# wizardyesterday/RtlSdrDiags

Measured on AMD Instinct MI355X. Metric: IQ MSamples/s through WBFM chain at 1/2/4/8 GPUs; % HBM roofline, higher is better.
Workload: dtype int8/int16 Q15 + f32; 1 GPU; BASELINE configs[1]: WBFM, 1 channel, 2^28-sample synthetic IQ; channels_per_gpu=1, log2_samples_per_channel=28, kernels=streaming pipelines

## Files before the change

### include/iqdemod.h

```cpp
#ifndef IQDEMOD_H
#define IQDEMOD_H

#include <stddef.h>
#include <stdint.h>

#ifdef __cplusplus
extern "C" {
#endif

#define IQD_ABI_VERSION 1

enum iqd_mode {
    IQD_MODE_NONE = 0, IQD_MODE_AM = 1, IQD_MODE_FM = 2,
    IQD_MODE_WBFM = 3, IQD_MODE_LSB = 4, IQD_MODE_USB = 5
};

enum iqd_demod { IQD_DEMOD_AM = 1, IQD_DEMOD_FM = 2, IQD_DEMOD_WBFM = 3, IQD_DEMOD_SSB = 4 };

enum iqd_status {
    IQD_OK = 0,
    IQD_EINVAL = -1,
    IQD_ENODEV = -2,
    IQD_ENOMEM = -3,
    IQD_EHIP = -4,
// ... 80 lines not shown

int iqd_demod_accept(iqd_t *e, uint32_t first_ch, uint32_t n_ch, int demod,
                     const int8_t *iq, size_t bytes_per_ch, int16_t *pcm);
int iqd_demod_set_sideband(iqd_t *e, uint32_t first_ch, uint32_t n_ch, int lsb);

int iqd_front_end(iqd_t *e, uint32_t first_ch, uint32_t n_ch, const uint8_t *iq, size_t bytes_per_ch, int8_t *out);
int iqd_front_end_device(iqd_t *e, uint32_t first_ch, uint32_t n_ch, const void *iq_dev, size_t bytes_per_ch,
                         void *out_dev);
int iqd_convert_fs_over_4(iqd_t *e, int direction, int8_t *buffer, size_t byte_count);

typedef struct iqd_stats {
    uint64_t accepts;
    uint64_t samples;
    uint64_t kernel_launches;
    uint64_t state_checks;
    uint64_t state_repairs;
    double chain_kernel_ms;
    uint64_t chain_kernel_count;
    uint64_t segment_repairs;
    uint64_t stream_launches;
    uint64_t device_launches;
    uint64_t device_copies;
    uint64_t mixed_launches;
} iqd_stats;

int iqd_get_stats(iqd_t *e, iqd_stats *out);
int iqd_set_profiling(iqd_t *e, int enabled);
int iqd_get_channel_mode(iqd_t *e, uint32_t ch, int *mode);
int iqd_get_channel_gain(iqd_t *e, uint32_t ch, int demod, float *gain);
const char *iqd_last_error(iqd_t *e);
const char *iqd_strerror(int status);
uint32_t iqd_abi_version(void);

enum iqd_resample_kind { IQD_RESAMPLE_DECIMATE_F32 = 0, IQD_RESAMPLE_INTERPOLATE_F32 = 1, IQD_RESAMPLE_INTERPOLATE_I16 = 2 };
typedef struct iqd_resampler iqd_resampler_t;
int iqd_resampler_create(iqd_t *e, int kind, const float *taps, uint32_t n_taps, uint32_t factor, uint32_t n_channels,
                         iqd_resampler_t **out);
void iqd_resampler_destroy(iqd_resampler_t *r);
int iqd_resampler_reset(iqd_resampler_t *r);
size_t iqd_resampler_out_count(const iqd_resampler_t *r, size_t n_in);
int iqd_resampler_run(iqd_resampler_t *r, const void *in, size_t n_in, void *out);
int iqd_resampler_run_device(iqd_resampler_t *r, const void *in_dev, size_t n_in, void *out_dev);

typedef struct iqd_channelizer_config {
    uint32_t n_sources;
    uint32_t n_channels;
// ... 53 lines not shown
```

### rtlsdrdiags_amd/capi.py

```python
import ctypes as C
import os
import weakref

import numpy as np

from .build import LIB as _DEFAULT_LIB

LIB = os.environ.get("IQD_LIB", _DEFAULT_LIB)

MODE = {"none": 0, "am": 1, "fm": 2, "wbfm": 3, "lsb": 4, "usb": 5}
DEMOD = {"am": 1, "fm": 2, "wbfm": 3, "ssb": 4}
F_NO_MAGNITUDE = 0x1
F_WBFM_TILES, F_WBFM_STREAM, F_PREPASS_OVERLAP = 0x2, 0x4, 0x8


class Config(C.Structure):
    _fields_ = [("abi_version", C.c_uint32), ("n_channels", C.c_uint32), ("block_bytes", C.c_uint32),
                ("device", C.c_int32), ("flags", C.c_uint32), ("reserved", C.c_uint32 * 3)]


class Stats(C.Structure):
    _fields_ = [("accepts", C.c_uint64), ("samples", C.c_uint64), ("kernel_launches", C.c_uint64),
                ("state_checks", C.c_uint64), ("state_repairs", C.c_uint64),
                ("chain_kernel_ms", C.c_double), ("chain_kernel_count", C.c_uint64), ("segment_repairs", C.c_uint64),
                ("stream_launches", C.c_uint64), ("device_launches", C.c_uint64), ("device_copies", C.c_uint64),
                ("mixed_launches", C.c_uint64)]


class AgcState(C.Structure):
    _fields_ = [("enabled", C.c_uint32), ("type", C.c_uint32), ("operating_point_dbfs", C.c_int32),
                ("deadband_db", C.c_uint32), ("blanking_limit", C.c_uint32), ("alpha", C.c_float),
                ("rx_gain_db", C.c_uint32), ("if_gain_db", C.c_uint32), ("filtered_if_gain_db", C.c_float),
                ("blanking_counter", C.c_uint32), ("gain_was_adjusted", C.c_uint32),
                ("normalized_level_dbfs", C.c_int32), ("signal_magnitude", C.c_uint32)]


class ChannelizerConfig(C.Structure):
    _fields_ = [("n_sources", C.c_uint32), ("n_channels", C.c_uint32), ("decimation", C.c_uint32),
                ("n_taps", C.c_uint32), ("taps", C.c_void_p), ("decimation_den", C.c_uint32),
                ("reserved", C.c_uint32 * 3)]


class IqdError(RuntimeError):
    def __init__(self, status, detail):
        super().__init__("libiqdemod: %s (%d): %s" % (_lib().iqd_strerror(status).decode(), status, detail))
        self.status = status


EXPORTS = [
# ... 552 lines not shown
```

### rtlsdrdiags_amd/csrc/iqd_accept.cpp

```cpp
#include "iqd_engine_impl.h"

extern "C" {


static void rebuild_lists(iqd_t *e, uint32_t first_ch, uint32_t n_ch)
{
    for (auto &l : e->h_lists) l.clear();
    e->any_gated = e->any_agc = false;
    for (uint32_t c = 0; c < n_ch; c++) {
        const ChanParams &p = e->h_params[first_ch + c];
        e->h_lists[family_of_mode(p.mode)].push_back(c);
        ChanParams worst = p;
        if (e->agc_touched[first_ch + c] && worst.rx_gain_db < AGC_MAX_GAIN) worst.rx_gain_db = AGC_MAX_GAIN;
        if (!squelch_always_open(worst, e->consts)) e->any_gated = true;
        if (e->h_agc[first_ch + c].enabled) e->any_agc = true;
    }
    for (int f = 0; f < FAM_COUNT; f++) {
        auto &l = e->h_lists[f];
        auto grp = [&](uint32_t c) { return 1 - e->h_params[first_ch + c].rotation; };
        std::stable_sort(l.begin(), l.end(), [&](uint32_t x, uint32_t y) { return grp(x) < grp(y); });
        for (int r = 0; r < 3; r++) e->rot_count[f][r] = 0;
        for (uint32_t c : l) e->rot_count[f][grp(c)]++;
    }
    e->list_first = first_ch;
// ... 4 lines not shown
namespace {
struct CallCtx {
    uint32_t first_ch = 0, n_ch = 0;
    const void *iq_dev = nullptr;
    size_t bytes_per_ch = 0;
    void *pcm_dev = nullptr, *pcm_count_dev = nullptr, *magnitude_dev = nullptr, *signal_present_dev = nullptr;
    uint32_t call_bb = 0, call_bs = 0, n_blocks = 0, vlen = 0;
    bool gated = false, any_agc = false, want_mag = false, pre_overlap = false, fused_mag = false;
    int pre_set = -1;
    DevBuf *gate_blk = nullptr, *gate_vlen = nullptr;
    SquelchLaunch q{};
    ChainLaunch base{};
    const CallPlan *plan = nullptr;
    hipStream_t s_main = nullptr;
    bool lane_used[4] = {false, false, false, false};
    bool timed = false, evp_open = false;
    std::pair<Event, Event> evp;
    MixedStreamArgs mix{};
    bool epoch_report_now = false;
    ChainLaunch tail_a{};
    int tail_f = 0;
    bool tail_pending = false;
    bool tail_dc = false;
};

int take_event_pair(iqd_t *e, CallCtx &x, hipStream_t s)
{
    if (e->ev_free_pairs.empty()) {
        Event a0, a1;
        HIP_TRY(e, hipEventCreate(a0.put()));
        HIP_TRY(e, hipEventCreate(a1.put()));
        e->ev_free_pairs.emplace_back(std::move(a0), std::move(a1));
    }
    x.evp = std::move(e->ev_free_pairs.back());
    e->ev_free_pairs.pop_back();
    HIP_TRY(e, hipEventRecord(x.evp.first, s));
    return IQD_OK;
}
}

static int prepare_call(iqd_t *e, CallCtx &x)
{
    hipStream_t s = e->stream;
    std::lock_guard<std::mutex> lk(e->mu);
    if (e->epoch_report_pending && ((volatile uint32_t *)e->h_epoch_report)[1] == e->epoch_report_seq) {
        if (((volatile uint32_t *)e->h_epoch_report)[0] == 0u)
// ... 172 lines not shown
    HIP_TRY(e, b8.ensure((size_t)x.n_ch * x.base.pcm_stride * sizeof(int32_t)));
    a.base8k = b8.as<int32_t>();
    a.dc_tiles = (uint32_t)((x.base.pcm_stride + DC_TILE - 1) / DC_TILE);
    DevBuf &dcr = f == FAM_SSB ? e->dc_records2 : e->dc_records;
    const size_t rec_bytes = (size_t)a.n_list * a.dc_tiles * sizeof(DcRecord);
    const bool grown = dcr.cap < rec_bytes + a.n_list * sizeof(uint32_t);
    HIP_TRY(e, dcr.ensure(rec_bytes + a.n_list * sizeof(uint32_t)));
    a.dc_records = dcr.p;
    size_t (&layout)[2] = e->dcr_layout[f == FAM_SSB];
    if (grown || layout[0] != rec_bytes || layout[1] < a.n_list) {
        HIP_COPY(e, hipMemsetAsync(dcr.as<char>() + rec_bytes, 0, a.n_list * sizeof(uint32_t), s));
        layout[0] = rec_bytes;
        layout[1] = a.n_list;
    }
    return IQD_OK;
}

static int queue_family(iqd_t *e, CallCtx &x, int f)
{
    const CallPlan &plan = *x.plan;
    const FamilyPlan &fp = plan.fam[f];
    const bool fused = plan.fused, forked = plan.forked, streams = fp.path == PLAN_STREAM;
    const uint32_t n_list = (uint32_t)e->h_lists[f].size();
    hipStream_t s = fp.lane == 0 ? x.s_main : e->fam_stream[fp.lane - 1];
    if (fp.lane != 0 && !x.lane_used[fp.lane]) HIP_TRY(e, hipStreamWaitEvent(s, e->fam_fork, 0));
    x.lane_used[fp.lane] = true;

    ChainLaunch a = x.base;
    a.ch_list = e->lists[f].as<uint32_t>();
    a.n_list = n_list;
    a.tile_len = fp.tile_len;
    a.tiles_per_ch = fp.tiles_per_ch;
    if (f == FAM_WBFM && x.gated && e->wbfm_epochs_live && !e->epoch_report_pending) {
        bool any = false;
        for (uint32_t c : e->h_lists[FAM_WBFM]) any = any || e->wbfm_epoch_left[x.first_ch + c] != 0;
        if (any) {
            if (!e->h_epoch_report) HIP_TRY(e, e->h_epoch_report.alloc(2));
            ((volatile uint32_t *)e->h_epoch_report)[0] = 0u;
            a.epoch_report = e->h_epoch_report;
            e->epoch_report_channels.clear();
            for (uint32_t c : e->h_lists[FAM_WBFM]) e->epoch_report_channels.push_back(x.first_ch + c);
            x.epoch_report_now = true;
        }
    }
    if (e->profiling && !x.timed && !fused) {
        int rc = take_event_pair(e, x, s);
// ... 16 lines not shown
            StreamArgs sa = e->stream_args;
            sa.amat = e->d_amat[stream_rot + 1];
            sa.half_lut = e->d_half_lut;
            sa.n_segments = n_list * a.tiles_per_ch;
            sa.grouped = fp.grouped ? 1u : 0u;
            for (int r = 0; r < 3; r++) {
                sa.group_start[r] = fp.grouped ? fp.group_start[r] : 0u;
                sa.group_li0[r] = fp.grouped ? fp.group_li0[r] : 0u;
                sa.group_nseg[r] = fp.grouped ? fp.group_nseg[r] : 0u;
                sa.amat3[r] = e->d_amat[2 - r];
            }
            sa.group_start[3] = fp.grouped ? fp.group_start[3] : 0u;
            sa.rounds = fp.rounds;
            sa.rings = fp.rings;
            HIP_TRY(e, e->stream_hist.ensure((size_t)sa.n_segments * sizeof(StHist)));
            sa.hist = e->stream_hist.as<StHist>();
            a.verify_at_end = x.gated ? 2u : 1u;
            if (fused) {
                x.mix.a[f] = a;
                x.mix.sa = sa;
                x.mix.wbfm_rot = stream_rot;
            } else {
                HIP_LAUNCH(e, launch_wbfm_stream(a, sa, stream_rot, x.fused_mag, fp.epochs, fp.grid, s));
                HIP_LAUNCH(e, launch_wbfm_stream_fixup(a, sa, s));
            }
            if (!x.gated) e->stream_handoffs += (uint64_t)n_list * ((x.vlen + a.tile_len - 1) / a.tile_len - 1);
            e->stats.stream_launches++;
        } else {
            HIP_LAUNCH(e, launch_wbfm(a, x.gated, x.fused_mag, n_list * a.tiles_per_ch, s));
        }
    } else {
        D4Args d4 = e->d4_args;
        if (streams) {
            for (int r = 0; r < 3; r++) {
                d4.group_start[r] = fp.group_start[r];
                d4.group_li0[r] = fp.group_li0[r];
                d4.group_nseg[r] = fp.group_nseg[r];
            }
            d4.group_start[3] = fp.group_start[3];
            d4.amat = e->d_amat4 + (size_t)(f == FAM_FM ? 0 : 3) * 4 * 64 * 4;
            d4.fm_lut = e->d_fmlut;
            d4.halo = (int32_t)fp.halo;
            d4.lead_shift = fp.lead_shift;
            d4.rounds = fp.rounds;
            d4.rings = fp.rings;
        }
        if (f != FAM_FM) {
// ... 16 lines not shown
                            (x.want_mag || x.pcm_count_dev || x.signal_present_dev || e->trace_on);
                if (f != FAM_FM && !x.tail_dc) HIP_LAUNCH(e, launch_am_dc(a, f, s, true));
            }
            e->stats.stream_launches++;
        } else if (f == FAM_FM) {
            HIP_LAUNCH(e, launch_fm(a, x.gated, x.fused_mag, n_list * a.tiles_per_ch, s));
        } else {
            HIP_LAUNCH(e, launch_am(a, f, x.gated, x.fused_mag, n_list * a.tiles_per_ch, s));
        }
    }
    if (e->profiling && !x.timed && !fused) {
        x.evp_open = true;
        x.timed = true;
    }
    e->stats.kernel_launches++;
    if (fused) return IQD_OK;
    if (f == FAM_WBFM && !x.gated && e->wbfm_epochs_live)
        for (uint32_t c : e->h_lists[FAM_WBFM]) {
            uint32_t &left = e->wbfm_epoch_left[x.first_ch + c];
            if (!left) continue;
            left = left > x.vlen ? left - x.vlen : 0u;
            if (!left) e->wbfm_epochs_live--;
        }
    const bool rides_with_squelch = !forked && !x.gated && !e->demod_bypass &&
                                    (x.want_mag || x.pcm_count_dev || x.signal_present_dev || e->trace_on);
    if (f == FAM_WBFM) {
        if (!streams) HIP_LAUNCH(e, launch_wbfm_verify(a, s));
        if (rides_with_squelch) {
            x.tail_a = a;
            x.tail_f = f;
            x.tail_pending = true;
        } else {
            HIP_LAUNCH(e, launch_wbfm_repair(a, x.gated, s));
        }
    } else if (rides_with_squelch) {
        x.tail_a = a;
        x.tail_f = f;
        x.tail_pending = true;
    } else {
        HIP_LAUNCH(e, launch_tail_update(a, f, s));
    }
    return IQD_OK;
}

static int queue_commit(iqd_t *e, CallCtx &x)
{
    const CallPlan &plan = *x.plan;
    hipStream_t s = x.s_main;
// ... 6 lines not shown
        e->stats.mixed_launches++;
        MixedTailArgs mt{};
        for (int f = 0; f < FAM_COUNT; f++) mt.a[f] = x.mix.a[f];
        mt.sa = x.mix.sa;
        HIP_LAUNCH(e, launch_mixed_tail(mt, s));
        if (e->profiling) x.evp_open = true;
        if (x.mix.a[FAM_WBFM].wg_count) {
            x.tail_a = x.mix.a[FAM_WBFM];
            x.tail_f = FAM_WBFM;
            x.tail_pending = true;
        }
    }
    for (int k = 1; k < 4; k++)
        if (x.lane_used[k]) {
            HIP_TRY(e, hipEventRecord(e->fam_join[k - 1], e->fam_stream[k - 1]));
            HIP_TRY(e, hipStreamWaitEvent(s, e->fam_join[k - 1], 0));
        }

    if (x.fused_mag && !e->h_lists[FAM_COUNT].empty())
        HIP_LAUNCH(e, launch_magnitude((const uint8_t *)x.iq_dev, x.bytes_per_ch, e->lists[FAM_COUNT].as<uint32_t>(),
                                    (uint32_t)e->h_lists[FAM_COUNT].size(), x.call_bs, x.n_blocks, e->mag_sums.as<uint32_t>(), s));
    if (!x.gated && !e->demod_bypass && (x.want_mag || x.pcm_count_dev || x.signal_present_dev || e->trace_on)) {
        x.q.zero_sums_after = x.any_agc ? 0u : 1u;
        HIP_LAUNCH(e, launch_squelch(x.q, true, s, x.tail_pending ? &x.tail_a : nullptr, x.tail_f, x.tail_pending && x.tail_dc));
        x.tail_pending = false;
        if (x.q.zero_sums_after) e->mag_sums_zero = (size_t)x.n_ch * x.n_blocks;
    }
    if (x.tail_pending) {
        if (x.tail_f == FAM_WBFM) HIP_LAUNCH(e, launch_wbfm_repair(x.tail_a, x.gated, s));
        else HIP_LAUNCH(e, launch_tail_update(x.tail_a, x.tail_f, s));
    }

    if (x.evp_open) {
        HIP_TRY(e, hipEventRecord(x.evp.second, s));
        e->ev_pending.push_back(std::move(x.evp));
    }
    if (x.pre_set >= 0) {
        HIP_TRY(e, hipEventRecord(e->ev_chain_done[x.pre_set], s));
        e->chain_pending[x.pre_set] = true;
    } else if (e->pre_stream && !e->demod_bypass) {
        HIP_TRY(e, hipEventRecord(e->ev_main_decisions, s));
        e->decisions_on_main = true;
    }
    if (x.epoch_report_now) {
        HIP_LAUNCH(e, launch_write_word(e->h_epoch_report + 1, e->accept_seq, s));
        e->epoch_report_pending = true;
        e->epoch_report_seq = e->accept_seq;
// ... 311 lines not shown
```

### rtlsdrdiags_amd/csrc/iqd_engine_impl.h

```cpp
#pragma once
#include "iqdemod.h"

#include <hip/hip_runtime.h>
#include <math.h>
#include <stdarg.h>
#include <stdio.h>
#include <string.h>

#include <algorithm>
#include <mutex>
#include <string>
#include <utility>
#include <vector>

#include "iqd_hipres.h"
#include "iqd_host.h"
#include "iqd_plan.h"
#include "iqd_kernels.h"
#include "iqd_stream.h"
#include "iqd_stream_mixed.h"
#include "iqd_taps.h"
#include "iqd_wbfm.h"
#include "iqd_chains.h"

// ... 48 lines not shown
    uint32_t wbfm_epochs_live = 0;
    std::vector<int32_t> rot_applied;
    bool rot_changed = false;
    DevArray<ScanConfig> d_scan_cfg;
    DevArray<ScanState> d_scan;
    DevArray<float> d_atan, d_fmlut;
    DevArray<float> d_half_lut;
    DevArray<uint32_t> d_amat[3];
    DevArray<uint32_t> d_amat4;
    D4Args d4_args{};
    std::vector<float> fm_kmax;
    bool stream_ok = false;
    std::vector<uint32_t> mode_gen, rot_gen;
    std::vector<float> wbfm_kmax;
    StreamArgs stream_args{};
    uint64_t stream_handoffs = 0;
    DevArray<uint32_t> d_counters;
    DevArray<unsigned long long> d_stamps;
    PinnedArray<uint32_t> h_counters;

    DevBuf stream_hist;
    DevBuf lists[FAM_COUNT + 1], mag_sums, blk_lists, vlen, records, base8k, base8k2, gain_trace, freq_trace, dc_records, dc_records2, repair_flags;
    size_t mag_sums_zero = 0;
    Stream pre_stream;
    Event ev_pre_done[2], ev_chain_done[2], ev_main_decisions;
    DevBuf g_sums[2], g_blk[2], g_vlen[2];
    int gate_set = 0;
    bool chain_pending[2] = {false, false};
    bool decisions_on_main = false;
    bool in_host_path = false;
    DevBuf st_iq, st_pcm, st_count, st_mag, st_allowed;
    DevBuf sl_iq[2], sl_pcm[2], sl_count[2], sl_mag[2], sl_allowed[2];
    Stream copy_stream;
    Stream fam_stream[3];
    Event fam_fork, fam_join[3];
    Event ev_in[2], ev_free[2];
    PinnedArray<uint32_t> h_slice_counts;
    DevArray<uint32_t> d_closed;
    PinnedArray<uint32_t> h_closed;
    PinnedArray<uint8_t> h_small;

    bool profiling = false;
    std::vector<std::pair<Event, Event>> ev_free_pairs, ev_pending;
    iqd_stats stats{};
    std::string last_error;

// ... 55 lines not shown
```

### rtlsdrdiags_amd/csrc/iqd_kernels.h

```cpp
#pragma once
#include <hip/hip_runtime.h>
#include <stddef.h>
#include <stdint.h>

#include "iqd_device.h"

namespace iqd {

struct WbfmStart;
struct WbfmRecord;

enum Counter { CNT_TILE_MISMATCH = 0, CNT_TILE_CHECKS = 1, CNT_SEG_REPAIRS = 2, CNT_DC_REDO = 3, CNT_TILE_REPAIRS = 4, CNT_STREAM_MISMATCH = 5, CNT_COUNT = 8 };
constexpr uint32_t MAX_MISMATCH_LIST = 1024;

struct ChainLaunch {
    const uint8_t *iq;
    size_t ch_stride_bytes;
    const uint32_t *ch_list;
    uint32_t n_list;
    uint32_t first_ch;
    uint32_t vlen;
    const uint32_t *vlen_gated;
    const uint32_t *blk_lists;
    uint32_t n_blocks;
// ... 60 lines not shown
struct StreamArgs;
hipError_t init_wbfm_stream_kernels();
hipError_t init_d4_stream_kernels();
hipError_t launch_wbfm_stream(const ChainLaunch &a, const StreamArgs &sa, int rotation, bool mag, bool epochs, uint32_t grid, hipStream_t s);
struct D4Args;
hipError_t launch_d4_stream(const ChainLaunch &a, const D4Args &da, int mode, bool mag, uint32_t grid, hipStream_t s);
hipError_t launch_am_dc(const ChainLaunch &a, int family, hipStream_t s, bool channel_major = false);
hipError_t launch_wbfm_stream_fixup(const ChainLaunch &a, const StreamArgs &sa, hipStream_t s);
hipError_t launch_retail(uint8_t *tails, const ChanParams *params, uint32_t n_ch, hipStream_t s);
hipError_t launch_resample(int kind, const void *in, void *out, const void *hist, void *hist_next, const void *taps,
                           uint32_t n_ch, uint32_t n_in, uint32_t n_out, uint32_t hist_len, uint32_t n_taps,
                           uint32_t factor, uint32_t first, hipStream_t s);
hipError_t launch_wbfm_repair(const ChainLaunch &a, bool gated, hipStream_t s);
hipError_t launch_front_end(const uint8_t *iq, int8_t *out, const ChanParams *params, uint32_t first_ch, uint32_t n_ch,
                            size_t bytes_per_ch, hipStream_t s);
hipError_t launch_rotate_signed(int8_t *buf_dev, size_t bytes, int rotation, hipStream_t s);
hipError_t launch_agc_apply(const AgcConfig *cfg, AgcState *st, const ScanConfig *scfg, ScanState *sst,
                            ChanParams *params, GainEpoch *epochs, uint32_t n_ch, hipStream_t s);
hipError_t launch_tail_update(const ChainLaunch &a, int family, hipStream_t s);
hipError_t launch_write_word(uint32_t *word, uint32_t value, hipStream_t s);
hipError_t launch_magnitude(const uint8_t *iq, size_t ch_stride_bytes, const uint32_t *ch_list, uint32_t n_list,
                            uint32_t block_samples, uint32_t n_blocks, uint32_t *mag_sums, hipStream_t s);
hipError_t launch_squelch(const SquelchLaunch &q, bool always_open, hipStream_t s, const ChainLaunch *tail_of = nullptr, int tail_family = 0, bool tail_dc = false);
hipError_t launch_tile_fill(uint8_t *dst, size_t period, size_t total, hipStream_t s);

}
```

### rtlsdrdiags_amd/csrc/iqd_kernels.hip

```cpp
#include <hip/hip_runtime.h>

#include "iqd_kernels.h"
#include "iqd_chains.h"
#include "iqd_wbfm.h"
#include "iqd_stream_fix.h"

namespace iqd {

__constant__ Consts g_consts;

hipError_t upload_consts(const Consts &c, hipStream_t s)
{
    return hipMemcpyToSymbolAsync(HIP_SYMBOL(g_consts), &c, sizeof(Consts), 0, hipMemcpyHostToDevice, s);
}

hipError_t consts_address(const Consts **p)
{
    void *a = nullptr;
    const hipError_t e = hipGetSymbolAddress(&a, HIP_SYMBOL(g_consts));
    *p = (const Consts *)a;
    return e;
}

struct DeviceExec {
// ... 101 lines not shown
#endif
template <bool GATED, bool MAG>
__global__ __launch_bounds__(WB_THREADS, IQD_WBFM_MIN_WAVES) void wbfm_chain_kernel(const ChainLaunch a)
{
    __shared__ WbfmLds lds;
    const uint32_t li = blockIdx.x / a.tiles_per_ch, tile = blockIdx.x - li * a.tiles_per_ch;
    const uint32_t ch = a.ch_list[li];
    const uint32_t vlen = GATED ? a.vlen_gated[ch] : a.vlen;
    if ((int64_t)tile * a.tile_len >= (int64_t)vlen) return;
    WbfmStart start;
    if (tile == 0) {
        const WbfmCarry cy = a.wbfm_carry[a.first_ch + ch];
        start.y = cy.y; start.u = cy.u; start.back = cy.back; start.cold = 0;
    } else {
        start.y = 0.f; start.u = 0.f; start.back = 0; start.cold = 1;
    }
    wbfm_run_tile<GATED, MAG>(a, lds, li, tile, ch, vlen, start);
}

__device__ __forceinline__ void tail_update_body(const ChainLaunch &a, int family, uint32_t li);
static_assert(WB_THREADS == 256, "the repair kernel ends with the tail update, which moves 16 bytes per thread");

template <bool GATED>
__device__ __forceinline__ void wbfm_repair_body(const ChainLaunch &a, WbfmLds &lds, const uint32_t li)
{
    const uint32_t ch = a.ch_list[li];
    const uint32_t vlen = GATED ? a.vlen_gated[ch] : a.vlen;
    const uint32_t ntiles = (vlen + a.tile_len - 1) / a.tile_len;
    if (a.verify_at_end == 2 && threadIdx.x == 0 && ntiles > 1) atomicAdd(&a.counters[CNT_TILE_CHECKS], ntiles - 1);
    if (!a.repair_flags[li]) {
        tail_update_body(a, FAM_WBFM, li);
        return;
    }
    WbfmRecord *r = a.records + (size_t)li * a.tiles_per_ch;
    const bool strong = a.params[a.first_ch + ch].wbfm_k >= 1.0f;
    __shared__ uint32_t first_bad;
    uint32_t from = 1;
    for (;;) {
        if (threadIdx.x == 0) first_bad = ntiles;
        __syncthreads();
        for (uint32_t tile = from + threadIdx.x; tile < ntiles; tile += blockDim.x)
            if (!iir_states_agree(r[tile].y_in, a.verify_at_end ? r[tile - 1].y_end : r[tile - 1].y_out, strong)) {
                atomicMin(&first_bad, tile);
                break;
            }
        __syncthreads();
        uint32_t tile = first_bad;
        __syncthreads();
        if (tile >= ntiles) break;
        bool redo_next = false;
        for (; tile < ntiles; tile++) {
            const WbfmRecord prev = r[tile - 1];
            const bool ok = iir_states_agree(r[tile].y_in, a.verify_at_end ? prev.y_end : prev.y_out, strong);
            if (ok && !redo_next) break;
            redo_next = a.verify_at_end && !ok;
            if (a.verify_at_end && tile + 2 == ntiles && vlen - (ntiles - 1) * a.tile_len < (uint32_t)FORCED_BACK) redo_next = true;
            WbfmStart start;
            start.y = prev.y_out; start.u = prev.u_out; start.back = prev.back_out; start.cold = 0;
            wbfm_run_tile<GATED, false>(a, lds, li, tile, ch, vlen, start);
            __threadfence();
            __syncthreads();
            if (threadIdx.x == 0) atomicAdd(&a.counters[CNT_TILE_REPAIRS], 1u);
        }
        from = tile;
        if (from >= ntiles) break;
    }
    if (threadIdx.x == 0) a.repair_flags[li] = 0;
    tail_update_body(a, FAM_WBFM, li);
}

template <bool GATED>
__global__ __launch_bounds__(WB_THREADS, IQD_WBFM_MIN_WAVES) void wbfm_repair_kernel(const ChainLaunch a)
{
    __shared__ WbfmLds lds;
    wbfm_repair_body<GATED>(a, lds, blockIdx.x);
}

__device__ __forceinline__ bool setup_tile(const ChainLaunch &a, bool gated, int family, Tile &t, uint32_t &ch, uint32_t &ech)
{
    const uint32_t li = blockIdx.x / a.tiles_per_ch, tile = blockIdx.x - li * a.tiles_per_ch;
    ch = a.ch_list[li];
    ech = a.first_ch + ch;
    const uint32_t vlen = gated ? a.vlen_gated[ch] : a.vlen;
    const int64_t v0 = (int64_t)tile * a.tile_len;
    if (v0 >= (int64_t)vlen) return false;
    const ChanParams &p = a.params[ech];
    t.iq_ch = a.iq + (size_t)ch * a.ch_stride_bytes;
    t.tail = a.tails + ((size_t)ech * FAM_COUNT + family) * TAIL_BYTES;
    t.blk_list = gated ? a.blk_lists + (size_t)ch * a.n_blocks : nullptr;
    t.block_samples = a.block_samples;
// ... 165 lines not shown
    }
}

__global__ void wbfm_verify_kernel(const ChainLaunch a)
{
    const uint32_t idx = blockIdx.x * blockDim.x + threadIdx.x;
    const uint32_t li = idx / a.tiles_per_ch, tile = idx % a.tiles_per_ch;
    if (li >= a.n_list) return;
    const uint32_t ch = a.ch_list[li];
    const uint32_t vlen = a.vlen_gated ? a.vlen_gated[ch] : a.vlen;
    const uint32_t ntiles = (vlen + a.tile_len - 1) / a.tile_len;
    if (tile >= ntiles) return;
    const WbfmRecord *r = a.records + (size_t)li * a.tiles_per_ch;
    if (tile > 0) {
        if (!iir_states_agree(r[tile].y_in, a.verify_at_end ? r[tile - 1].y_end : r[tile - 1].y_out, a.params[a.first_ch + ch].wbfm_k >= 1.0f)) {
            atomicAdd(&a.counters[CNT_TILE_MISMATCH], 1u);
            a.repair_flags[li] = 1;
        } else {
            atomicAdd(&a.counters[CNT_TILE_CHECKS], 1u);
        }
    }
}

__device__ __forceinline__ void tail_update_body(const ChainLaunch &a, int family, uint32_t li)
{
    const uint32_t ch = a.ch_list[li];
    const uint32_t ech = a.first_ch + ch;
    const uint32_t vlen = a.vlen_gated ? a.vlen_gated[ch] : a.vlen;
    if (family == FAM_WBFM && a.epoch_report && threadIdx.x == 0 &&
        (uint64_t)a.epochs[ech].wbfm.since[0] + vlen < (uint64_t)TAIL)
        *(volatile uint32_t *)a.epoch_report = 1u;
    if (vlen == 0) return;
    if (family == FAM_WBFM && threadIdx.x == 0) {
        const uint32_t ntiles = (vlen + a.tile_len - 1) / a.tile_len;
        const WbfmRecord r = a.records[(size_t)li * a.tiles_per_ch + ntiles - 1];
        const WbfmRecord p = a.records[(size_t)li * a.tiles_per_ch + (ntiles >= 2 ? ntiles - 2 : 0)];
        a.wbfm_carry[ech] = wbfm_pick_carry(r, p, ntiles, vlen, a.tile_len, a.verify_at_end);
    }
    if (threadIdx.x < EPOCHS && (family == FAM_WBFM || family == FAM_FM)) {
        uint32_t *since = (family == FAM_WBFM ? a.epochs[ech].wbfm.since : a.epochs[ech].fm.since) + threadIdx.x;
        const uint64_t total = (uint64_t)*since + vlen;
        *since = total < (uint64_t)TAIL ? (uint32_t)total : (uint32_t)TAIL;
    }
    uint8_t *tail = a.tails + ((size_t)ech * FAM_COUNT + family) * TAIL_BYTES;
    const uint8_t *iq_ch = a.iq + (size_t)ch * a.ch_stride_bytes;
    const uint32_t *blk_list = a.vlen_gated ? a.blk_lists + (size_t)ch * a.n_blocks : nullptr;
    const int keep = family == FAM_WBFM ? tail_keep(FAM_WBFM) : family == FAM_FM ? tail_keep(FAM_FM) : family == FAM_AM ? tail_keep(FAM_AM) : tail_keep(FAM_SSB);
    const bool mine = 8 * (int)threadIdx.x < keep;
    const int64_t v = (int64_t)vlen - keep + 8 * (int64_t)(mine ? threadIdx.x : 0);
    const uint8_t *src;
    if (v < 0) src = tail + TAIL_BYTES + 2 * v;
    else if (!blk_list) src = iq_ch + 2 * v;
    else {
        const uint32_t blk = (uint32_t)(v / a.block_samples);
        const uint32_t off = (uint32_t)(v - (int64_t)blk * a.block_samples);
        src = iq_ch + ((int64_t)blk_list[blk] * a.block_samples + off) * 2;
    }
    uint4 val{};
    if (mine) val = *(const uint4 *)src;
    __syncthreads();
#ifndef IQD_NO_WT_STORES
// ... 60 lines not shown
{
    if (blockIdx.x < a.n_list) tail_update_body(a, family, blockIdx.x);
    else squelch_block_body(q, always_open, (blockIdx.x - a.n_list) * 256u + threadIdx.x);
}

__global__ __launch_bounds__(256) void tail_dc_squelch_kernel(const ChainLaunch a, int family, const SquelchLaunch q, int always_open)
{
    __shared__ DcLds lds;
    if (blockIdx.x < a.n_list) {
        if (threadIdx.x >= 64) return;
        dc_channel_wave(a, family, blockIdx.x, lds);
    } else if (blockIdx.x < 2 * a.n_list) {
        tail_update_body(a, family, blockIdx.x - a.n_list);
    } else {
        squelch_block_body(q, always_open, (blockIdx.x - 2 * a.n_list) * 256u + threadIdx.x);
    }
}

__global__ __launch_bounds__(WB_THREADS, IQD_WBFM_MIN_WAVES) void wbfm_repair_squelch_kernel(const ChainLaunch a, const SquelchLaunch q, int always_open)
{
    __shared__ WbfmLds lds;
    if (blockIdx.x < a.n_list) wbfm_repair_body<false>(a, lds, blockIdx.x);
    else squelch_block_body(q, always_open, (blockIdx.x - a.n_list) * 256u + threadIdx.x);
}

struct MixedTailRoles { uint32_t end[6]; };
__global__ __launch_bounds__(256) void mixed_tail_kernel(const ChainLaunch a_wbfm, const StreamArgs sa, const ChainLaunch a_am,
                                                         const ChainLaunch a_fm, const ChainLaunch a_ssb, const MixedTailRoles roles)
{
    __shared__ union Lds { DcLds dc; FixLds fix; __device__ Lds() {} } u;
    DcLds &lds = u.dc;
    const uint32_t b = blockIdx.x;
    if (b < roles.end[0]) {
        wbfm_stream_fixup_body(a_wbfm, sa, b, u.fix);
    } else if (b < roles.end[2]) {
        if (threadIdx.x >= 64) return;
        const int family = b < roles.end[1] ? FAM_AM : FAM_SSB;
        const ChainLaunch &a = family == FAM_AM ? a_am : a_ssb;
        const uint32_t li = b - (family == FAM_AM ? roles.end[0] : roles.end[1]);
        dc_channel_wave(a, family, li, lds);
    } else if (b < roles.end[3]) {
        tail_update_body(a_am, FAM_AM, b - roles.end[2]);
    } else if (b < roles.end[4]) {
        tail_update_body(a_fm, FAM_FM, b - roles.end[3]);
    } else if (b < roles.end[5]) {
        tail_update_body(a_ssb, FAM_SSB, b - roles.end[4]);
// ... 445 lines not shown
}

hipError_t launch_tail_update(const ChainLaunch &a, int family, hipStream_t s)
{
    hipLaunchKernelGGL(tail_update_kernel, dim3(a.n_list), dim3(256), 0, s, a, family);
    return hipGetLastError();
}

__global__ void write_word_kernel(uint32_t *word, uint32_t value) { *(volatile uint32_t *)word = value; }
hipError_t launch_write_word(uint32_t *word, uint32_t value, hipStream_t s)
{
    hipLaunchKernelGGL(write_word_kernel, dim3(1), dim3(1), 0, s, word, value);
    return hipGetLastError();
}

hipError_t launch_magnitude(const uint8_t *iq, size_t ch_stride_bytes, const uint32_t *ch_list, uint32_t n_list,
                            uint32_t block_samples, uint32_t n_blocks, uint32_t *mag_sums, hipStream_t s)
{
    hipLaunchKernelGGL(magnitude_kernel, dim3(n_blocks, n_list), dim3(256), 0, s, iq, ch_stride_bytes, ch_list,
                       block_samples, n_blocks, mag_sums);
    return hipGetLastError();
}

hipError_t launch_squelch(const SquelchLaunch &q, bool always_open, hipStream_t s, const ChainLaunch *tail_of, int tail_family, bool tail_dc)
{
    const uint32_t n = q.n_ch * q.n_blocks;
    if (tail_of && tail_dc)
        hipLaunchKernelGGL(tail_dc_squelch_kernel, dim3(2 * tail_of->n_list + (n + 255) / 256), dim3(256), 0, s, *tail_of, tail_family, q, always_open ? 1 : 0);
    else if (tail_of && tail_family == FAM_WBFM)
        hipLaunchKernelGGL(wbfm_repair_squelch_kernel, dim3(tail_of->n_list + (n + 255) / 256), dim3(WB_THREADS), 0, s, *tail_of, q, always_open ? 1 : 0);
    else if (tail_of)
        hipLaunchKernelGGL(tail_squelch_kernel, dim3(tail_of->n_list + (n + 255) / 256), dim3(256), 0, s, *tail_of, tail_family, q, always_open ? 1 : 0);
    else
        hipLaunchKernelGGL(squelch_block_kernel, dim3((n + 255) / 256), dim3(256), 0, s, q, always_open ? 1 : 0);
    if (!always_open || q.any_agc) {
        if (q.n_blocks >= 32)
            hipLaunchKernelGGL(squelch_track_wave_kernel, dim3(q.n_ch), dim3(64), 0, s, q, always_open ? 1 : 0);
        else
            hipLaunchKernelGGL(squelch_track_kernel, dim3((q.n_ch + 63) / 64), dim3(64), 0, s, q, always_open ? 1 : 0);
    }
    return hipGetLastError();
}

hipError_t launch_mixed_tail(const MixedTailArgs &m, hipStream_t s)
{
    MixedTailRoles roles;
    uint32_t at = 0;
    if (m.a[FAM_WBFM].wg_count) at += (m.sa.n_segments + FIX_SEGS - 1) / FIX_SEGS;
    roles.end[0] = at;
    if (m.a[FAM_AM].wg_count) at += m.a[FAM_AM].n_list;
    roles.end[1] = at;
    if (m.a[FAM_SSB].wg_count) at += m.a[FAM_SSB].n_list;
    roles.end[2] = at;
    if (m.a[FAM_AM].wg_count) at += m.a[FAM_AM].n_list;
    roles.end[3] = at;
    if (m.a[FAM_FM].wg_count) at += m.a[FAM_FM].n_list;
    roles.end[4] = at;
    if (m.a[FAM_SSB].wg_count) at += m.a[FAM_SSB].n_list;
    roles.end[5] = at;
    if (at) hipLaunchKernelGGL(mixed_tail_kernel, dim3(at), dim3(256), 0, s, m.a[FAM_WBFM], m.sa, m.a[FAM_AM], m.a[FAM_FM], m.a[FAM_SSB], roles);
    return hipGetLastError();
}

// ... 47 lines not shown
```

### rtlsdrdiags_amd/csrc/iqd_plan.cpp

```cpp
#include "iqd_plan.h"

#include <algorithm>

#include "iqdemod.h"
#include "iqd_stream.h"

namespace iqd {

uint64_t stream_min_seg(const PlanKnobs &k, int f, uint64_t vlen, int several_families)
{
    if (k.env_stream_min_seg) return k.env_stream_min_seg;
    if (several_families == 2) return STREAM_MIN_SEG_FORKED;
    if (several_families) return vlen < 8192 ? STREAM_MIN_SEG_MIXED_SHORT : STREAM_MIN_SEG_MIXED;
    if (f == FAM_WBFM) return STREAM_MIN_SEG_WBFM;
    if (f == FAM_FM) return STREAM_MIN_SEG_FM;
    if (f == FAM_AM) return vlen <= 16384 ? STREAM_MIN_SEG_AM_SHORT : STREAM_MIN_SEG_AM;
    return vlen <= 16384 ? STREAM_MIN_SEG_SSB_SHORT : STREAM_MIN_SEG_SSB;
}

namespace {

uint32_t halo_of(int f, uint32_t shift)
{
    return f == FAM_WBFM ? (uint32_t)ST_HALO : (uint32_t)d4_full_halo(f) - shift;
}

uint32_t group_ids(const FamilyShape &s, FamilyPlan &p)
{
    uint32_t at = 0, li0 = 0;
    for (int r = 0; r < 3; r++) {
        p.group_start[r] = at;
        p.group_li0[r] = li0;
        p.group_nseg[r] = s.rot_count[r] * p.tiles_per_ch;
        at += (p.group_nseg[r] + 15u) / 16u * 16u;
        li0 += s.rot_count[r];
    }
    p.group_start[3] = at;
    return at;
}

// ... 153 lines not shown
                    }
                    if (!shift || k.d4_leadfree >= 0 || p.tiles_per_ch >= D4_LEADFREE_MIN_TILES) break;
                    shift = 0;
                }
            }
        }
        if (fused) {
            if (p.path != PLAN_STREAM) return false;
            p.wg_first = out.mix_wgs;
            out.mix_wgs += p.grid;
        }
    }
    return true;
}

}

void plan_call(const PlanKnobs &k, const CallShape &c, CallPlan &out)
{
    if (!plan_once(k, c, true, out)) plan_once(k, c, false, out);
}

}
```

### rtlsdrdiags_amd/csrc/iqd_stream.h

```cpp
#pragma once
#include <stdint.h>

#include "iqd_device.h"

namespace iqd {

constexpr int ST_WAVES = 15;
constexpr int ST_THREADS = 64 * ST_WAVES;
constexpr int ST_RINGS = 3;
constexpr int ST_P_PER_RING = 4;
constexpr int ST_SEGS = 64 * ST_RINGS;
constexpr int ST_HALO = FORCED_BACK;
#ifndef IQD_ST_AHEAD
#define IQD_ST_AHEAD 2
#endif
constexpr int ST_AHEAD = IQD_ST_AHEAD;
constexpr int ST_MIN_TILE = 768;
constexpr int ST_FIX_PCM = 21;
constexpr int ST_ROW_FLOATS = 260;
#ifndef IQD_ST_FAKE_SHIFT
#define IQD_ST_FAKE_SHIFT 0
#endif
constexpr int ST_LDS_ROW_FLOATS = IQD_ST_FAKE_SHIFT ? (256 >> IQD_ST_FAKE_SHIFT) + 4 : ST_ROW_FLOATS;
constexpr int ST_TABLE_BYTES = 129 * ST_LDS_ROW_FLOATS * 4;
// ... 18 lines not shown
    uint32_t y2_last[20];
};
static_assert(sizeof(StHist) == 256, "one boundary record per segment, 256 bytes");

struct StreamArgs {
    StHist *hist;
    const uint32_t *amat;
    const float *half_lut;
    uint32_t n_segments;
    uint32_t rounds;
    uint32_t rings;
    uint32_t grouped;
    uint32_t group_start[4];
    uint32_t group_li0[3];
    uint32_t group_nseg[3];
    const uint32_t *amat3[3];
    uint32_t d1p[4];
    uint32_t d1p2[4];
    uint32_t p12p[6];
    uint32_t a40p[20];
    float b0, a1;
};

enum { D4_AM = 0, D4_SSB = 1, D4_FM = 2 };
constexpr int D4_HALO_AM = fir_halo(FAM_AM), D4_HALO_SSB = fir_halo(FAM_SSB), D4_HALO_FM = fir_halo(FAM_FM);
constexpr int D4_HALO_SHORT = 128;
constexpr int d4_full_halo(int family) { return family == FAM_FM ? D4_HALO_FM : family == FAM_AM ? D4_HALO_AM : D4_HALO_SSB; }
constexpr int d4_lead_shift(int family) { return d4_full_halo(family) - D4_HALO_SHORT; }
constexpr int D4_REPLAY_AM = 4, D4_REPLAY_SSB = 36, D4_REPLAY_FM = 20;
constexpr int D4_REPLAY_PAIRS_AMSSB = 4;
constexpr int D4_RAILS_FROM_PIECE = 8;
constexpr int d4_replay_outputs(int family) { return family == FAM_FM ? D4_REPLAY_FM : family == FAM_AM ? D4_REPLAY_AM : D4_REPLAY_SSB; }
struct D4Geom { int64_t v0; uint32_t skip, cold; };
#if defined(__HIPCC__)
__host__ __device__
#endif
inline D4Geom d4_geom(uint32_t sid, uint32_t tile, uint32_t tile_len, uint32_t shift)
{
    D4Geom g;
    if (!shift) { g.v0 = (int64_t)tile * tile_len; g.skip = 0; g.cold = 1; return g; }
    g.cold = tile == 0 || (sid & 63u) == 0 ? 1u : 0u;
    const uint32_t c = 1u + (sid >> 6) - ((sid - tile) >> 6);
    g.v0 = (int64_t)tile * tile_len - (int64_t)shift * c;
    g.skip = g.cold ? shift : 0u;
    return g;
}
// ... 24 lines not shown
```

### rtlsdrdiags_amd/csrc/iqd_stream_fix.h

```cpp
#pragma once
#include <hip/hip_runtime.h>

#include "iqd_kernels.h"
#include "iqd_stream.h"
#include "iqd_stream_mixed.h"
#include "iqd_wbfm.h"
#include "iqd_mfma.h"

namespace iqd {

struct StSeg {
    uint32_t valid, li, tile, ch, ech;
    int32_t v0, tlen;
    int32_t vlen;
};

__device__ __forceinline__ StSeg st_segment(const ChainLaunch &a, uint32_t sid, uint32_t n_segments)
{
    StSeg s;
    s.valid = sid < n_segments ? 1u : 0u;
    const uint32_t id = s.valid ? sid : 0u;
    s.li = id / a.tiles_per_ch;
    s.tile = id - s.li * a.tiles_per_ch;
    s.ch = a.ch_list[s.li];
// ... 73 lines not shown
#pragma unroll
        for (int k = 0; k < 4; k++) y1[k] = prev.y1_last[k];
#pragma unroll
        for (int k = 0; k < 6; k++) y1[4 + k] = own.y1_first[k];
        y1[4] = (y1[4] & 0xffff0000u) | ((uint32_t)(acc >> 15) & 0xffffu);
        int s2 = 1 << 14;
#pragma unroll
        for (int q = 0; q < 6; q++) {
            const uint32_t d = i == 0 ? y1[5 - q] : (i == 1 ? y1[7 - q] : y1[9 - q]);
            s2 = dot2(d, sa.p12p[q], s2);
        }
        ((int16_t *)&y2x[sl][20])[i] = (int16_t)(s2 >> 15);
    } else if (live) {
        for (int p = i - 3; p < 41; p += FIX_LANES - 3) {
            if (p == 20) continue;
            if (p == 21) ((int16_t *)&y2x[sl][21])[1] = (int16_t)(own.y2_first[1] >> 16);
            else y2x[sl][p] = p < 20 ? prev.y2_last[p] : own.y2_first[p - 20];
        }
    }
    if (live && i == FIX_LANES - 1 && f2u(y_in) != f2u(y_end)) {
        if (!iir_states_agree(y_in, y_end, a.params[sg.ech].wbfm_k >= 1.0f)) {
            atomicAdd(&a.counters[CNT_TILE_MISMATCH], 1u);
            atomicAdd(&a.counters[CNT_STREAM_MISMATCH], 1u);
            a.repair_flags[sg.li] = 1;
        }
    }
    __syncthreads();
    if (!live) return;
    for (int j = i; j < ST_FIX_PCM && j < sg.tlen / 32; j += FIX_LANES) {
        int s3 = 1 << 14;
#pragma unroll
        for (int q = 0; q < 20; q++) {
            const uint32_t pair = y2x[sl][20 + j - q];
            s3 = clamp_q30(dot2(pair, sa.a40p[q] & 0xffff0000u, s3));
            s3 = clamp_q30(dot2(pair, sa.a40p[q] & 0x0000ffffu, s3));
        }
        a.pcm[(size_t)sg.ch * a.pcm_stride + (sg.v0 >> 5) + j] = (int16_t)(s3 >> 15);
    }
}

}
```

Before: 829,300 MSamples/s.

## Fuse WBFM stream fixup, tail update and squelch into one closing kernel

For up to eight WBFM channels where a squelch pass follows, the separate stream fixup launch and the squelch/tail launch are merged into one kernel. Workgroups take fixup, tail-update or squelch roles, and a striped atomic arrival counter picks the last workgroup. That workgroup re-runs the repair walk against saved old tails when any channel was flagged. This removes a kernel launch and its inter-kernel gap per call, at the cost of extra atomics, a tail snapshot store, and a serial repair path in a single workgroup when repair is needed.

```diff
diff --git a/include/iqdemod.h b/include/iqdemod.h
--- a/include/iqdemod.h
+++ b/include/iqdemod.h
@@ -126,6 +126,7 @@
     uint64_t device_launches;
     uint64_t device_copies;
     uint64_t mixed_launches;
+    uint64_t closed_in_fixup;
 } iqd_stats;
 
 int iqd_get_stats(iqd_t *e, iqd_stats *out);
diff --git a/rtlsdrdiags_amd/capi.py b/rtlsdrdiags_amd/capi.py
--- a/rtlsdrdiags_amd/capi.py
+++ b/rtlsdrdiags_amd/capi.py
@@ -24,7 +24,7 @@
                 ("state_checks", C.c_uint64), ("state_repairs", C.c_uint64),
                 ("chain_kernel_ms", C.c_double), ("chain_kernel_count", C.c_uint64), ("segment_repairs", C.c_uint64),
                 ("stream_launches", C.c_uint64), ("device_launches", C.c_uint64), ("device_copies", C.c_uint64),
-                ("mixed_launches", C.c_uint64)]
+                ("mixed_launches", C.c_uint64), ("closed_in_fixup", C.c_uint64)]
 
 
 class AgcState(C.Structure):
diff --git a/rtlsdrdiags_amd/csrc/iqd_accept.cpp b/rtlsdrdiags_amd/csrc/iqd_accept.cpp
--- a/rtlsdrdiags_amd/csrc/iqd_accept.cpp
+++ b/rtlsdrdiags_amd/csrc/iqd_accept.cpp
@@ -50,6 +50,8 @@
     int tail_f = 0;
     bool tail_pending = false;
     bool tail_dc = false;
+    bool close_in_fixup = false;
+    StreamArgs close_sa{};
 };
 
 int take_event_pair(iqd_t *e, CallCtx &x, hipStream_t s)
@@ -268,6 +270,8 @@
     const FamilyPlan &fp = plan.fam[f];
     const bool fused = plan.fused, forked = plan.forked, streams = fp.path == PLAN_STREAM;
     const uint32_t n_list = (uint32_t)e->h_lists[f].size();
+    const bool rides_with_squelch = !forked && !x.gated && !e->demod_bypass &&
+                                    (x.want_mag || x.pcm_count_dev || x.signal_present_dev || e->trace_on);
     hipStream_t s = fp.lane == 0 ? x.s_main : e->fam_stream[fp.lane - 1];
     if (fp.lane != 0 && !x.lane_used[fp.lane]) HIP_TRY(e, hipStreamWaitEvent(s, e->fam_fork, 0));
     x.lane_used[fp.lane] = true;
@@ -330,7 +334,9 @@
                 x.mix.wbfm_rot = stream_rot;
             } else {
                 HIP_LAUNCH(e, launch_wbfm_stream(a, sa, stream_rot, x.fused_mag, fp.epochs, fp.grid, s));
-                HIP_LAUNCH(e, launch_wbfm_stream_fixup(a, sa, s));
+                x.close_in_fixup = rides_with_squelch && n_list <= WBFM_CLOSE_MAX_CH;
+                if (x.close_in_fixup) x.close_sa = sa;
+                else HIP_LAUNCH(e, launch_wbfm_stream_fixup(a, sa, s));
             }
             if (!x.gated) e->stream_handoffs += (uint64_t)n_list * ((x.vlen + a.tile_len - 1) / a.tile_len - 1);
             e->stats.stream_launches++;
@@ -393,8 +399,6 @@
             left = left > x.vlen ? left - x.vlen : 0u;
             if (!left) e->wbfm_epochs_live--;
         }
-    const bool rides_with_squelch = !forked && !x.gated && !e->demod_bypass &&
-                                    (x.want_mag || x.pcm_count_dev || x.signal_present_dev || e->trace_on);
     if (f == FAM_WBFM) {
         if (!streams) HIP_LAUNCH(e, launch_wbfm_verify(a, s));
         if (rides_with_squelch) {
@@ -447,7 +451,17 @@
                                     (uint32_t)e->h_lists[FAM_COUNT].size(), x.call_bs, x.n_blocks, e->mag_sums.as<uint32_t>(), s));
     if (!x.gated && !e->demod_bypass && (x.want_mag || x.pcm_count_dev || x.signal_present_dev || e->trace_on)) {
         x.q.zero_sums_after = x.any_agc ? 0u : 1u;
-        HIP_LAUNCH(e, launch_squelch(x.q, true, s, x.tail_pending ? &x.tail_a : nullptr, x.tail_f, x.tail_pending && x.tail_dc));
+        if (x.close_in_fixup) {
+            if (!e->d_close_words) {
+                HIP_TRY(e, e->d_close_words.alloc(CLOSE_WORDS));
+                HIP_TRY(e, e->d_tails_old.alloc((size_t)e->n_ch * FAM_COUNT * TAIL_BYTES));
+                HIP_COPY(e, hipMemsetAsync(e->d_close_words, 0, CLOSE_WORDS * sizeof(uint32_t), s));
+            }
+            HIP_LAUNCH(e, launch_wbfm_fixup_close(x.tail_a, x.close_sa, x.q, true, e->d_close_words, e->d_tails_old, s));
+            e->stats.closed_in_fixup++;
+        } else {
+            HIP_LAUNCH(e, launch_squelch(x.q, true, s, x.tail_pending ? &x.tail_a : nullptr, x.tail_f, x.tail_pending && x.tail_dc));
+        }
         x.tail_pending = false;
         if (x.q.zero_sums_after) e->mag_sums_zero = (size_t)x.n_ch * x.n_blocks;
     }
diff --git a/rtlsdrdiags_amd/csrc/iqd_engine_impl.h b/rtlsdrdiags_amd/csrc/iqd_engine_impl.h
--- a/rtlsdrdiags_amd/csrc/iqd_engine_impl.h
+++ b/rtlsdrdiags_amd/csrc/iqd_engine_impl.h
@@ -94,6 +94,8 @@
     DevBuf stream_hist;
     DevBuf lists[FAM_COUNT + 1], mag_sums, blk_lists, vlen, records, base8k, base8k2, gain_trace, freq_trace, dc_records, dc_records2, repair_flags;
     size_t mag_sums_zero = 0;
+    DevArray<uint32_t> d_close_words;
+    DevArray<uint8_t> d_tails_old;
     Stream pre_stream;
     Event ev_pre_done[2], ev_chain_done[2], ev_main_decisions;
     DevBuf g_sums[2], g_blk[2], g_vlen[2];
diff --git a/rtlsdrdiags_amd/csrc/iqd_kernels.h b/rtlsdrdiags_amd/csrc/iqd_kernels.h
--- a/rtlsdrdiags_amd/csrc/iqd_kernels.h
+++ b/rtlsdrdiags_amd/csrc/iqd_kernels.h
@@ -106,6 +106,8 @@
 hipError_t launch_magnitude(const uint8_t *iq, size_t ch_stride_bytes, const uint32_t *ch_list, uint32_t n_list,
                             uint32_t block_samples, uint32_t n_blocks, uint32_t *mag_sums, hipStream_t s);
 hipError_t launch_squelch(const SquelchLaunch &q, bool always_open, hipStream_t s, const ChainLaunch *tail_of = nullptr, int tail_family = 0, bool tail_dc = false);
+hipError_t launch_wbfm_fixup_close(const ChainLaunch &a, const StreamArgs &sa, const SquelchLaunch &q, bool always_open,
+                                   uint32_t *words, uint8_t *tails_old, hipStream_t s);
 hipError_t launch_tile_fill(uint8_t *dst, size_t period, size_t total, hipStream_t s);
 
 }
diff --git a/rtlsdrdiags_amd/csrc/iqd_kernels.hip b/rtlsdrdiags_amd/csrc/iqd_kernels.hip
--- a/rtlsdrdiags_amd/csrc/iqd_kernels.hip
+++ b/rtlsdrdiags_amd/csrc/iqd_kernels.hip
@@ -147,16 +147,11 @@
 static_assert(WB_THREADS == 256, "the repair kernel ends with the tail update, which moves 16 bytes per thread");
 
 template <bool GATED>
-__device__ __forceinline__ void wbfm_repair_body(const ChainLaunch &a, WbfmLds &lds, const uint32_t li)
+__device__ __forceinline__ void wbfm_repair_walk(const ChainLaunch &a, WbfmLds &lds, const uint32_t li)
 {
     const uint32_t ch = a.ch_list[li];
     const uint32_t vlen = GATED ? a.vlen_gated[ch] : a.vlen;
     const uint32_t ntiles = (vlen + a.tile_len - 1) / a.tile_len;
-    if (a.verify_at_end == 2 && threadIdx.x == 0 && ntiles > 1) atomicAdd(&a.counters[CNT_TILE_CHECKS], ntiles - 1);
-    if (!a.repair_flags[li]) {
-        tail_update_body(a, FAM_WBFM, li);
-        return;
-    }
     WbfmRecord *r = a.records + (size_t)li * a.tiles_per_ch;
     const bool strong = a.params[a.first_ch + ch].wbfm_k >= 1.0f;
     __shared__ uint32_t first_bad;
@@ -191,6 +186,20 @@
         if (from >= ntiles) break;
     }
     if (threadIdx.x == 0) a.repair_flags[li] = 0;
+}
+
+template <bool GATED>
+__device__ __forceinline__ void wbfm_repair_body(const ChainLaunch &a, WbfmLds &lds, const uint32_t li)
+{
+    const uint32_t ch = a.ch_list[li];
+    const uint32_t vlen = GATED ? a.vlen_gated[ch] : a.vlen;
+    const uint32_t ntiles = (vlen + a.tile_len - 1) / a.tile_len;
+    if (a.verify_at_end == 2 && threadIdx.x == 0 && ntiles > 1) atomicAdd(&a.counters[CNT_TILE_CHECKS], ntiles - 1);
+    if (!a.repair_flags[li]) {
+        tail_update_body(a, FAM_WBFM, li);
+        return;
+    }
+    wbfm_repair_walk<GATED>(a, lds, li);
     tail_update_body(a, FAM_WBFM, li);
 }
 
@@ -402,6 +411,19 @@
     }
 }
 
+__device__ __forceinline__ void wbfm_commit_carry(const ChainLaunch &a, uint32_t li, uint32_t ech, uint32_t vlen)
+{
+    const uint32_t ntiles = (vlen + a.tile_len - 1) / a.tile_len;
+    const WbfmRecord r = a.records[(size_t)li * a.tiles_per_ch + ntiles - 1];
+    const WbfmRecord p = a.records[(size_t)li * a.tiles_per_ch + (ntiles >= 2 ? ntiles - 2 : 0)];
+    const WbfmCarry cy = wbfm_pick_carry(r, p, ntiles, vlen, a.tile_len, a.verify_at_end);
+    static_assert(sizeof(WbfmCarry) == 32, "four 8-byte stores");
+    const unsigned long long *src = (const unsigned long long *)&cy;
+    unsigned long long *dst = (unsigned long long *)&a.wbfm_carry[ech];
+#pragma unroll
+    for (int k = 0; k < 4; k++) __hip_atomic_store(dst + k, src[k], __ATOMIC_RELAXED, __HIP_MEMORY_SCOPE_AGENT);
+}
+
 __device__ __forceinline__ void tail_update_body(const ChainLaunch &a, int family, uint32_t li)
 {
     const uint32_t ch = a.ch_list[li];
@@ -411,12 +433,7 @@
         (uint64_t)a.epochs[ech].wbfm.since[0] + vlen < (uint64_t)TAIL)
         *(volatile uint32_t *)a.epoch_report = 1u;
     if (vlen == 0) return;
-    if (family == FAM_WBFM && threadIdx.x == 0) {
-        const uint32_t ntiles = (vlen + a.tile_len - 1) / a.tile_len;
-        const WbfmRecord r = a.records[(size_t)li * a.tiles_per_ch + ntiles - 1];
-        const WbfmRecord p = a.records[(size_t)li * a.tiles_per_ch + (ntiles >= 2 ? ntiles - 2 : 0)];
-        a.wbfm_carry[ech] = wbfm_pick_carry(r, p, ntiles, vlen, a.tile_len, a.verify_at_end);
-    }
+    if (family == FAM_WBFM && threadIdx.x == 0) wbfm_commit_carry(a, li, ech, vlen);
     if (threadIdx.x < EPOCHS && (family == FAM_WBFM || family == FAM_FM)) {
         uint32_t *since = (family == FAM_WBFM ? a.epochs[ech].wbfm.since : a.epochs[ech].fm.since) + threadIdx.x;
         const uint64_t total = (uint64_t)*since + vlen;
@@ -523,6 +540,69 @@
     __shared__ WbfmLds lds;
     if (blockIdx.x < a.n_list) wbfm_repair_body<false>(a, lds, blockIdx.x);
     else squelch_block_body(q, always_open, (blockIdx.x - a.n_list) * 256u + threadIdx.x);
+}
+
+struct FixupCloseArgs {
+    uint32_t *words;
+    uint8_t *tails_old;
+    uint32_t n_fix;
+};
+__global__ __launch_bounds__(WB_THREADS, 3) void wbfm_fixup_close_kernel(const ChainLaunch a, const StreamArgs sa, const SquelchLaunch q,
+                                                                  int always_open, const FixupCloseArgs c)
+{
+    static_assert(FIX_THREADS == WB_THREADS && FIX_THREADS * 16 == TAIL_BYTES, "one role per workgroup, 16 bytes of a tail per thread");
+    static_assert(3 * sizeof(WbfmLds) <= 160 * 1024, "three workgroups per CU: the LDS, and the registers by the launch bounds");
+    __shared__ union Lds { WbfmLds wb; FixLds fix; __device__ Lds() {} } u;
+    __shared__ uint32_t last_arriver;
+    const uint32_t b = blockIdx.x;
+    if (b < c.n_fix) {
+        wbfm_stream_fixup_body(a, sa, b, u.fix);
+    } else if (b < c.n_fix + a.n_list) {
+        const uint32_t li = b - c.n_fix;
+        const size_t slot = ((size_t)(a.first_ch + a.ch_list[li]) * FAM_COUNT + FAM_WBFM) * TAIL_BYTES;
+        const uint4 old = ((const uint4 *)(a.tails + slot))[threadIdx.x];
+        {
+            typedef uint32_t wt4 __attribute__((ext_vector_type(4)));
+            const wt4 vv = {old.x, old.y, old.z, old.w};
+            const void *dst = c.tails_old + slot + 16 * (int)threadIdx.x;
+            asm volatile("global_store_dwordx4 %0, %1, off sc1\n\ts_nop 1" :: "v"(dst), "v"(vv) : "memory");
+        }
+        __syncthreads();
+        tail_update_body(a, FAM_WBFM, li);
+    } else {
+        squelch_block_body(q, always_open, (b - c.n_fix - a.n_list) * 256u + threadIdx.x);
+    }
+    asm volatile("s_waitcnt vmcnt(0)" ::: "memory");
+    __syncthreads();
+    if (threadIdx.x == 0) {
+        uint32_t last = 0;
+        const uint32_t stripe = b % CLOSE_STRIPES;
+        uint32_t *w = c.words + stripe * CLOSE_WORD_STRIDE, *top = c.words + CLOSE_STRIPES * CLOSE_WORD_STRIDE;
+        if (atomicAdd(w, 1u) + 1u == close_stripe_target(gridDim.x, stripe)) {
+            atomicExch(w, 0u);
+            if (atomicAdd(top, 1u) + 1u == (gridDim.x < CLOSE_STRIPES ? gridDim.x : CLOSE_STRIPES)) {
+                atomicExch(top, 0u);
+                last = 1;
+                for (uint32_t li = 0; li < a.n_list; li++)
+                    last |= __hip_atomic_load(&a.repair_flags[li], __ATOMIC_RELAXED, __HIP_MEMORY_SCOPE_AGENT) ? 2u : 0u;
+            }
+        }
+        last_arriver = last;
+    }
+    __syncthreads();
+    if (last_arriver < 2) return;
+    __builtin_amdgcn_fence(__ATOMIC_ACQUIRE, "agent");
+    asm volatile("s_waitcnt vmcnt(0)" ::: "memory");
+    __syncthreads();
+    ChainLaunch old_tails = a;
+    old_tails.tails = c.tails_old;
+    for (uint32_t li = 0; li < a.n_list; li++) {
+        if (!__hip_atomic_load(&a.repair_flags[li], __ATOMIC_RELAXED, __HIP_MEMORY_SCOPE_AGENT)) continue;
+        wbfm_repair_walk<false>(old_tails, u.wb, li);
+        const uint32_t ch = a.ch_list[li];
+        if (threadIdx.x == 0 && a.vlen) wbfm_commit_carry(a, li, a.first_ch + ch, a.vlen);
+        __syncthreads();
+    }
 }
 
 struct MixedTailRoles { uint32_t end[6]; };
@@ -1014,6 +1094,15 @@
     return hipGetLastError();
 }
 
+static void launch_squelch_tracking(const SquelchLaunch &q, bool always_open, hipStream_t s)
+{
+    if (always_open && !q.any_agc) return;
+    if (q.n_blocks >= 32)
+        hipLaunchKernelGGL(squelch_track_wave_kernel, dim3(q.n_ch), dim3(64), 0, s, q, always_open ? 1 : 0);
+    else
+        hipLaunchKernelGGL(squelch_track_kernel, dim3((q.n_ch + 63) / 64), dim3(64), 0, s, q, always_open ? 1 : 0);
+}
+
 hipError_t launch_squelch(const SquelchLaunch &q, bool always_open, hipStream_t s, const ChainLaunch *tail_of, int tail_family, bool tail_dc)
 {
     const uint32_t n = q.n_ch * q.n_blocks;
@@ -1025,12 +1114,21 @@
         hipLaunchKernelGGL(tail_squelch_kernel, dim3(tail_of->n_list + (n + 255) / 256), dim3(256), 0, s, *tail_of, tail_family, q, always_open ? 1 : 0);
     else
         hipLaunchKernelGGL(squelch_block_kernel, dim3((n + 255) / 256), dim3(256), 0, s, q, always_open ? 1 : 0);
-    if (!always_open || q.any_agc) {
-        if (q.n_blocks >= 32)
-            hipLaunchKernelGGL(squelch_track_wave_kernel, dim3(q.n_ch), dim3(64), 0, s, q, always_open ? 1 : 0);
-        else
-            hipLaunchKernelGGL(squelch_track_kernel, dim3((q.n_ch + 63) / 64), dim3(64), 0, s, q, always_open ? 1 : 0);
-    }
+    launch_squelch_tracking(q, always_open, s);
+    return hipGetLastError();
+}
+
+hipError_t launch_wbfm_fixup_close(const ChainLaunch &a, const StreamArgs &sa, const SquelchLaunch &q, bool always_open,
+                                   uint32_t *words, uint8_t *tails_old, hipStream_t s)
+{
+    FixupCloseArgs c;
+    c.words = words;
+    c.tails_old = tails_old;
+    c.n_fix = (sa.n_segments + FIX_SEGS - 1) / FIX_SEGS;
+    const uint32_t n = q.n_ch * q.n_blocks;
+    hipLaunchKernelGGL(wbfm_fixup_close_kernel, dim3(c.n_fix + a.n_list + (n + 255) / 256), dim3(FIX_THREADS), 0, s, a, sa, q,
+                       always_open ? 1 : 0, c);
+    launch_squelch_tracking(q, always_open, s);
     return hipGetLastError();
 }
 
diff --git a/rtlsdrdiags_amd/csrc/iqd_plan.cpp b/rtlsdrdiags_amd/csrc/iqd_plan.cpp
--- a/rtlsdrdiags_amd/csrc/iqd_plan.cpp
+++ b/rtlsdrdiags_amd/csrc/iqd_plan.cpp
@@ -16,6 +16,16 @@
     if (f == FAM_FM) return STREAM_MIN_SEG_FM;
     if (f == FAM_AM) return vlen <= 16384 ? STREAM_MIN_SEG_AM_SHORT : STREAM_MIN_SEG_AM;
     return vlen <= 16384 ? STREAM_MIN_SEG_SSB_SHORT : STREAM_MIN_SEG_SSB;
+}
+
+uint32_t close_stripe_targets(uint32_t grid, uint32_t *targets)
+{
+    uint32_t active = 0;
+    for (uint32_t s = 0; s < CLOSE_STRIPES; s++) {
+        targets[s] = close_stripe_target(grid, s);
+        active += targets[s] ? 1u : 0u;
+    }
+    return active;
 }
 
 namespace {
@@ -215,3 +225,5 @@
 }
 
 }
+
+extern "C" uint32_t iqd_plan_close_stripe_targets(uint32_t grid, uint32_t *targets) { return iqd::close_stripe_targets(grid, targets); }
diff --git a/rtlsdrdiags_amd/csrc/iqd_stream.h b/rtlsdrdiags_amd/csrc/iqd_stream.h
--- a/rtlsdrdiags_amd/csrc/iqd_stream.h
+++ b/rtlsdrdiags_amd/csrc/iqd_stream.h
@@ -64,6 +64,19 @@
     float b0, a1;
 };
 
+constexpr uint32_t WBFM_CLOSE_MAX_CH = 8;
+constexpr uint32_t CLOSE_STRIPES = 64;
+constexpr uint32_t CLOSE_WORD_STRIDE = 32;
+constexpr uint32_t CLOSE_WORDS = (CLOSE_STRIPES + 1) * CLOSE_WORD_STRIDE;
+#if defined(__HIPCC__)
+__host__ __device__
+#endif
+inline uint32_t close_stripe_target(uint32_t grid, uint32_t stripe)
+{
+    return grid / CLOSE_STRIPES + (stripe < grid % CLOSE_STRIPES ? 1u : 0u);
+}
+uint32_t close_stripe_targets(uint32_t grid, uint32_t *targets );
+
 enum { D4_AM = 0, D4_SSB = 1, D4_FM = 2 };
 constexpr int D4_HALO_AM = fir_halo(FAM_AM), D4_HALO_SSB = fir_halo(FAM_SSB), D4_HALO_FM = fir_halo(FAM_FM);
 constexpr int D4_HALO_SHORT = 128;
diff --git a/rtlsdrdiags_amd/csrc/iqd_stream_fix.h b/rtlsdrdiags_amd/csrc/iqd_stream_fix.h
--- a/rtlsdrdiags_amd/csrc/iqd_stream_fix.h
+++ b/rtlsdrdiags_amd/csrc/iqd_stream_fix.h
@@ -119,7 +119,7 @@
         if (!iir_states_agree(y_in, y_end, a.params[sg.ech].wbfm_k >= 1.0f)) {
             atomicAdd(&a.counters[CNT_TILE_MISMATCH], 1u);
             atomicAdd(&a.counters[CNT_STREAM_MISMATCH], 1u);
-            a.repair_flags[sg.li] = 1;
+            atomicOr(&a.repair_flags[sg.li], 1u);
         }
     }
     __syncthreads();
@@ -132,7 +132,7 @@
             s3 = clamp_q30(dot2(pair, sa.a40p[q] & 0xffff0000u, s3));
             s3 = clamp_q30(dot2(pair, sa.a40p[q] & 0x0000ffffu, s3));
         }
-        a.pcm[(size_t)sg.ch * a.pcm_stride + (sg.v0 >> 5) + j] = (int16_t)(s3 >> 15);
+        __hip_atomic_store(&a.pcm[(size_t)sg.ch * a.pcm_stride + (sg.v0 >> 5) + j], (int16_t)(s3 >> 15), __ATOMIC_RELAXED, __HIP_MEMORY_SCOPE_AGENT);
     }
 }
 
```

Result: slower. 809,900 MSamples/s (-2.3%).
